# EspressoSystems/Push-CDN

Measured on NVIDIA H100. Metric: broadcast fan-out egress GB/s (1 KiB x 2^20 subscribers per GPU, 1 topic); msgs/s and % of HBM peak alongside, higher is better.
Workload: dtype u8

## Files before the change

push-cdn_b200/csrc/kernels.cu:

```cuda
#include "kernels.cuh"

#include <atomic>

#include "frame_parse_core.h"

namespace pcdn {

std::atomic<unsigned long long> g_kernel_launches{0};
#define PCDN_COUNT_LAUNCH (void)g_kernel_launches.fetch_add(1, std::memory_order_relaxed)

unsigned long long kernel_launches() { return g_kernel_launches.load(std::memory_order_relaxed); }
void count_kernel_launch() { PCDN_COUNT_LAUNCH; }

__device__ __forceinline__ uint32_t lane_id() { return threadIdx.x & 31; }

__device__ __forceinline__ uint32_t warp_incl_scan(uint32_t v) {
  const uint32_t lane = lane_id();
#pragma unroll
  for (int o = 1; o < 32; o <<= 1) {
    uint32_t n = __shfl_up_sync(0xffffffffu, v, o);
    if (lane >= (uint32_t)o) v += n;
  }
  return v;
}
// ... 649 lines not shown
      }
    } else if (threadIdx.x == 0) {
      cta_prefix = 0;
      w.lb_tot[vb] = ctot;
    }
    __syncthreads();
    k.s1_off = cta_prefix + cex;
    w.cbase[c] = k.s1_off;
  } else {
    s.ptail[c] = k.pt;
    s.used[c] = k.us;
  }
  w.batch_units[c] = k.bu;

  const uint32_t nsp = (k.s1_rec ? 1u : 0u) + (k.s2_rec ? 1u : 0u);
  uint32_t tot, ex;
  uint32_t run_len = 1, my_runs = nsp, nsp_warp = 0;
  if (s.span_runs) {
    __shared__ uint32_t r_off[NT], r_len[NT], r_rec[NT], r_brk[NT + 1];
    const uint32_t t = threadIdx.x;
    r_off[t] = k.s1_off; r_len[t] = k.s1_units; r_rec[t] = nsp == 1 ? k.s1_rec : 0u;
    __syncthreads();
    const bool cont = t > 0 && nsp == 1 && r_rec[t - 1] == k.s1_rec && r_len[t - 1] == k.s1_units &&
                      (s.pool ? r_off[t - 1] + r_len[t - 1] == k.s1_off : r_off[t - 1] == k.s1_off);
    const uint32_t head = (nsp > 0 && !cont) ? 1u : 0u;
    my_runs = head ? nsp : 0u;
    uint32_t ptot;
    const uint32_t pex = cta_excl_scan<NW>(my_runs | (cont ? 0u : 1u << 16), &ptot, sm);
    ex = pex & 0xFFFFu; tot = ptot & 0xFFFFu;
    const uint32_t brk = pex >> 16;
    if (!cont) r_brk[brk] = t;
    if (t == 0) r_brk[ptot >> 16] = NT;
    __syncthreads();
    if (head) run_len = r_brk[brk + 1] - t;
    if (threadIdx.x == 0) span_base = tot ? atomicAdd(&w.stats->n_runs, tot) : 0;
    nsp_warp = __reduce_add_sync(0xffffffffu, nsp);
  } else {
    ex = cta_excl_scan<NW>(nsp, &tot, sm);
    if (threadIdx.x == 0) span_base = tot ? atomicAdd(&w.stats->n_spans, tot) : 0;
  }
  const unsigned long long nrec = __reduce_add_sync(0xffffffffu, k.s1_rec + k.s2_rec);
  const unsigned long long by = (unsigned long long)__reduce_add_sync(0xffffffffu, k.bytes & 0xFFFFu) +
                                ((unsigned long long)__reduce_add_sync(0xffffffffu, k.bytes >> 16) << 16);
  if (lane == 0) { red[0][threadIdx.x >> 5] = nrec | ((unsigned long long)nsp_warp << 48); red[1][threadIdx.x >> 5] = by; }
  __syncthreads();
  if (threadIdx.x == 0) {
    unsigned long long a = 0, bb = 0, sp = 0;
    for (int i = 0; i < NW; i++) { a += red[0][i] & 0xFFFFFFFFFFFFull; sp += red[0][i] >> 48; bb += red[1][i]; }
    if (a) { atomicAdd(&w.stats->n_deliveries, a); atomicAdd(&w.stats->bytes_out, bb); }
    if (sp) atomicAdd(&w.stats->n_spans, (uint32_t)sp);
  }
  if (s.span_runs) {
    if (my_runs) {
      SpanRun* runs = reinterpret_cast<SpanRun*>(w.spans);
      uint32_t at = span_base + ex;
      if (k.s1_rec) runs[at++] = SpanRun{s.conn_base + c, run_len, s.pool ? k.s1_off : k.s1_off * kUnit, k.s1_units * kUnit, k.s1_rec, s.pool ? k.s1_units : 0u};
      if (k.s2_rec) runs[at] = SpanRun{s.conn_base + c, 1, 0, k.s2_units * kUnit, k.s2_rec, 0};
    }
  } else if (nsp) {
    uint32_t at = span_base + ex;
    if (k.s1_rec) w.spans[at++] = Span{s.conn_base + c, s.pool ? k.s1_off : k.s1_off * kUnit, k.s1_units * kUnit, k.s1_rec};
    if (k.s2_rec) w.spans[at] = Span{s.conn_base + c, 0, k.s2_units * kUnit, k.s2_rec};
  }
  if (k.ovf) {
    uint32_t i = atomicAdd(&w.stats->n_overflow, 1u);
    if (i < max_conns) w.overflow[i] = s.conn_base + c;
  }
}
template <bool HAS_DIRECT>
__global__ void __launch_bounds__(256) k_offsets(DevState s, BatchIn b, Work w, uint32_t max_conns) {
  offsets_body<HAS_DIRECT, 256, false, false>(s, b, w, max_conns, blockIdx.x * 256 + threadIdx.x, blockIdx.x, gridDim.x);
}
__global__ void __launch_bounds__(1024) k_pool_finish(DevState s, Work w, uint32_t nblk) {
  extern __shared__ uint32_t tb[];
  __shared__ uint32_t sm[33];
  __shared__ unsigned long long total_s;
  if (w.stats->status) return;
  unsigned long long carry = 0;
  for (uint32_t b0 = 0; b0 < nblk; b0 += 1024) {
    const uint32_t i = b0 + threadIdx.x;
    const uint32_t v = i < nblk ? w.lb_tot[i] : 0;
    uint32_t tot, ex = cta_excl_scan<32>(v, &tot, sm);
    const unsigned long long at = carry + ex;
    if (i < nblk) tb[i] = at > 0xFFFFFFFFull ? 0xFFFFFFFFu : (uint32_t)at;
    carry += tot;
  }
  if (threadIdx.x == 0) total_s = carry;
  __syncthreads();
  if (blockIdx.x == 0 && threadIdx.x == 0) pool_allocate(s, w, total_s);
  const uint32_t gt = blockIdx.x * 1024 + threadIdx.x, gn = gridDim.x * 1024;
  for (uint32_t c = gt; c < s.N; c += gn) w.cbase[c] += tb[c >> 8];
  if (s.span_runs) {
    SpanRun* r = reinterpret_cast<SpanRun*>(w.spans);
    const uint32_t n = w.stats->n_runs;
    for (uint32_t i = gt; i < n; i += gn) r[i].ring_off += tb[(r[i].conn0 - s.conn_base) >> 8];
  } else {
    const uint32_t n = w.stats->n_spans;
    for (uint32_t i = gt; i < n; i += gn) w.spans[i].ring_off += tb[(w.spans[i].conn - s.conn_base) >> 8];
  }
}

void launch_offsets(const DevState& s, const Work& w, const BatchIn& b, bool has_direct, int n_sms, cudaStream_t st) {
  if (has_direct) PCDN_COUNT_LAUNCH, k_offsets<true><<<s.N / 256, 256, 0, st>>>(s, b, w, s.N);
  else PCDN_COUNT_LAUNCH, k_offsets<false><<<s.N / 256, 256, 0, st>>>(s, b, w, s.N);
  if (s.pool) {
    const uint32_t nblk = s.N / 256;
    if (nblk * 4 > 48u * 1024) cudaFuncSetAttribute(k_pool_finish, cudaFuncAttributeMaxDynamicSharedMemorySize, (int)(nblk * 4));
    PCDN_COUNT_LAUNCH, k_pool_finish<<<std::min<uint32_t>((uint32_t)n_sms, (s.N + 8191) / 8192), 1024, nblk * 4, st>>>(s, w, nblk);
  }
}

__device__ __forceinline__ void cluster_sync_all() {
  asm volatile("barrier.cluster.arrive.release.aligned;\n\tbarrier.cluster.wait.acquire.aligned;" ::: "memory");
}
template <bool HAS_DIRECT>
__global__ void __cluster_dims__(8, 1, 1) __launch_bounds__(1024, 1)
k_ctrl_small(DevState s, BatchIn b, Work w, int zero_stats, BatchStats* publish, int offsets_only) {
  __shared__ uint32_t sm[33];
  __shared__ uint32_t gbase[5];
  const uint32_t tid = threadIdx.x, rank = blockIdx.x;
  if (zero_stats && rank == 0 && tid < sizeof(BatchStats) / 4) reinterpret_cast<uint32_t*>(w.stats)[tid] = 0;

  if (HAS_DIRECT && rank == 0 && !offsets_only) {
    __shared__ uint32_t skey_s[kSmallCtrlMsgs], sorted_s[kSmallCtrlMsgs];
    __syncthreads();
    for (uint32_t g0 = 0; g0 < b.n_msgs * 8; g0 += 1024) direct_lookup_body<false>(s, b, w, g0 + tid);
    __syncthreads();
    const uint32_t n = b.n_msgs;
    if (tid < n) { const uint32_t t = w.dconn[tid]; skey_s[tid] = t == kConnNone ? s.N : t; }
    __syncthreads();
    if (tid < n) {
      const uint32_t key = skey_s[tid];
      uint32_t r = 0;
      for (uint32_t o = 0; o < n; o++) r += (skey_s[o] < key || (skey_s[o] == key && o < tid)) ? 1u : 0u;
      sorted_s[r] = key;
      w.dlist[r] = tid;
    }
    __syncthreads();
    if (tid < n) {
      const uint32_t key = sorted_s[tid];
      if (tid == 0 || sorted_s[tid - 1] != key) { w.dstart[key] = tid; w.dstamp[key] = w.stamp; }
      if (tid + 1 == n || sorted_s[tid + 1] != key) w.dend[key] = tid + 1;
    }
  }

  if (!offsets_only) {
    const uint32_t q = tid >> 8, wl = tid & 255u, nitems = b.n_bcast * s.nblk;
    for (uint32_t i0 = rank * 4; i0 < nitems; i0 += 32) {
      const uint32_t it = i0 + q;
      const bool live = it < nitems;
      const uint32_t j = live ? it / s.nblk : 0, blk = live ? it % s.nblk : 0;
      const uint32_t wd = blk * kBlockWords + wl;
      const uint32_t word = live ? match_word(s, b, b.bcast_index[j], wd) : 0;
      uint32_t tot, ex = cta_excl_scan<32>(__popc(word), &tot, sm);
      if (wl == 0) gbase[q] = ex;
      if (tid == 0) gbase[4] = tot;
      __syncthreads();
      if (live) {
        w.B[(size_t)j * s.W + wd] = word;
        w.wpre[(size_t)j * s.W + wd] = (uint16_t)(ex - gbase[q]);
        if (wl == 0) w.cnt[(size_t)j * s.nblk + blk] = gbase[q + 1] - gbase[q];
      }
      __syncthreads();
    }
  }
  cluster_sync_all();

  if (rank == 0 && !offsets_only) {
    if (tid < b.n_bcast) {
      uint32_t carry = 0;
      for (uint32_t blk = 0; blk < s.nblk; blk++) {
        const uint32_t v = w.cnt[(size_t)tid * s.nblk + blk];
        w.base[(size_t)tid * s.nblk + blk] = carry;
        carry += v;
      }
      const uint32_t m = b.bcast_index[tid];
      w.D[m] = carry; w.jidx[m] = tid;
    }
    __syncthreads();
  }

  if (rank == 0 && !offsets_only) {
    const uint32_t m = tid;
    const bool valid = m < b.n_msgs;
    const uint32_t d = valid ? w.D[m] : 0;
    uint32_t cls, tiles;
    plan_classify(s, b, m, d, &cls, &tiles);
    uint32_t t0, t1, t2, t3;
    const uint32_t e0 = cta_excl_scan<32>(cls != CLS_THIN ? d : 0, &t0, sm);
    const uint32_t e1 = cta_excl_scan<32>(cls == CLS_THIN ? d : 0, &t1, sm);
    const uint32_t e2 = cta_excl_scan<32>(tiles, &t2, sm);
    const uint32_t e3 = cta_excl_scan<32>(cls == CLS_CM ? 1u : 0u, &t3, sm);
    if (valid) {
      w.eb_fat[m] = e0; w.eb_thin[m] = e1; w.tbase[m] = e2; w.cm_rank[m] = e3; w.cls[m] = (uint8_t)cls;
      if (cls == CLS_CM) w.cm_list[e3] = m;
    }
    if (tid == 0) {
      w.stats->n_fat_entries = t0; w.stats->n_thin_entries = t1; w.stats->n_fat_tiles = t2; w.stats->tile_cursor = 0;
      w.stats->n_cm = t3; w.stats->cm_cursor = 0;
      if (t0 > w.cap_fat || t1 > w.cap_thin) w.stats->status = 1;
      const uint32_t n = b.n_msgs;
      w.eb_fat[n] = t0; w.eb_thin[n] = t1; w.tbase[n] = t2; w.cm_rank[n] = t3;
    }
  }
  cluster_sync_all();

  for (uint32_t c0 = 0; c0 < s.N; c0 += 8192)
    offsets_body<HAS_DIRECT, 1024, true, true>(s, b, w, s.N, c0 + rank * 1024 + tid, c0 / 1024 + rank, s.N / 1024);

  if (publish) {
    cluster_sync_all();
    if (rank == 0 && tid < sizeof(BatchStats) / 4)
      reinterpret_cast<uint32_t*>(publish)[tid] = __ldcg(reinterpret_cast<const uint32_t*>(w.stats) + tid);
  }
}
void launch_ctrl_small(const DevState& s, const Work& w, const BatchIn& b, bool has_direct, bool zero_stats,
                       BatchStats* publish, bool offsets_only, cudaStream_t st) {
  if (has_direct) PCDN_COUNT_LAUNCH, k_ctrl_small<true><<<8, 1024, 0, st>>>(s, b, w, zero_stats ? 1 : 0, publish, offsets_only ? 1 : 0);
  else PCDN_COUNT_LAUNCH, k_ctrl_small<false><<<8, 1024, 0, st>>>(s, b, w, zero_stats ? 1 : 0, publish, offsets_only ? 1 : 0);
}

__global__ void k_pool_retry_begin(BatchStats* bs) {
  bs->status = 0;
  bs->n_deliveries = 0; bs->bytes_out = 0;
  bs->n_spans = 0; bs->n_runs = 0; bs->n_overflow = 0;
  bs->tile_cursor = 0; bs->cm_cursor = 0;
}
void launch_pool_retry_begin(const DevState& s, const Work& w, cudaStream_t st) {
  cudaMemsetAsync(w.lb_state, 0, ((size_t)s.N / 256 + 1) * 8, st);
  PCDN_COUNT_LAUNCH, k_pool_retry_begin<<<1, 1, 0, st>>>(w.stats);
}

__device__ __forceinline__ uint8_t* conn_out(const DevState& s, const Work& w, uint32_t conn, uint32_t pool_base) {
  return s.pool ? s.rings + ((size_t)pool_base + w.cbase[conn]) * kUnit : s.rings + (size_t)conn * s.ring_bytes;
}

__device__ __forceinline__ void pack_fat_phase(const DevState& s, const BatchIn& b, const Work& w, uint8_t* buf,
                                               uint64_t* barp) {
  uint64_t& bar = *barp;
  __shared__ uint32_t t_info[8];
  const uint32_t tid = threadIdx.x;
  const uint32_t ntiles = w.stats->n_fat_tiles;
  if (ntiles == 0) return;
  const uint32_t pool_base = w.stats->pool_base;
  uint32_t phase = 0;
  uint32_t staged_m = 0xFFFFFFFFu, staged_k = 0xFFFFFFFFu;

  for (;;) {
    if (tid == 0) {
      const uint32_t t = atomicAdd(&w.stats->tile_cursor, 1u);
      t_info[0] = t;
      if (t < ntiles) {
        uint32_t lo = 0, hi = b.n_msgs;
        while (hi - lo > 1) { uint32_t mid = (lo + hi) >> 1; if (w.tbase[mid] <= t) lo = mid; else hi = mid; }
        const uint32_t m = lo, ltile = t - w.tbase[m], d = w.D[m];
        const uint32_t fb = frame_vec_bytes(b.raw_len[m]);
        const uint32_t tr = tile_recipients(fb);
        const uint32_t ngrp = (d + tr - 1) / tr;
        const uint32_t ch = ltile / ngrp, grp = ltile % ngrp;
        const uint32_t nbytes = min(kChunkBytes, fb - ch * kChunkBytes);
        t_info[1] = m; t_info[2] = ch; t_info[3] = grp * tr;
        t_info[4] = min(d, (grp + 1) * tr); t_info[5] = nbytes;
        t_info[6] = (m != staged_m || ch != staged_k) ? 1u : 0u;
        staged_m = m; staged_k = ch;
      }
    }
    __syncthreads();
    if (t_info[0] >= ntiles) break;
    const uint32_t m = t_info[1], ch = t_info[2], r0 = t_info[3], r1 = t_info[4], nbytes = t_info[5];
    if (t_info[6]) {
      bulk_wait_read0();
      __syncthreads();
      if (tid == 0) {
        mbar_arrive_expect_tx(&bar, nbytes);
        bulk_g2s(buf, b.arena + (size_t)b.slot_off16[m] * 16 + (size_t)ch * kChunkBytes, nbytes, &bar);
      }
      mbar_wait(&bar, phase);
      phase ^= 1;
      if (ch == 0) {
        if (tid == 0) {
          *reinterpret_cast<uint32_t*>(buf) = bswap32(b.raw_len[m]);
          fence_proxy_async_smem();
        }
        __syncthreads();
      }
    }
    const uint2* E = w.efat + w.eb_fat[m];
    const size_t chunk_off = (size_t)ch * kChunkBytes;
    for (uint32_t r = r0 + tid; r < r1; r += 256) {
      const uint2 ent = E[r];
      if (ent.y != kOffInvalid)
        bulk_s2g(conn_out(s, w, ent.x, pool_base) + (size_t)ent.y * kUnit + chunk_off, buf, nbytes);
    }
    bulk_commit();
    __syncthreads();
  }
  bulk_wait_read0();
}

__device__ __forceinline__ void pack_cm_phase(const DevState& s, const BatchIn& b, const Work& w, uint8_t* buf,
                                              uint64_t* barp) {
  uint64_t& bar = *barp;
  __shared__ uint32_t g_m[kCmGroup], g_j[kCmGroup], g_soff[kCmGroup], g_units[kCmGroup], g_eb[kCmGroup];
  __shared__ uint32_t t_info[4];
  const uint32_t tid = threadIdx.x, lane = tid & 31, warp = tid >> 5;
  if (w.stats->status) return;
  const uint32_t ncm = w.stats->n_cm;
  if (ncm == 0) return;
  const uint32_t pool_base = w.stats->pool_base;
  const uint32_t ngroups = (ncm + kCmGroup - 1) / kCmGroup;
  const uint32_t tpg = s.W / kCmTileWords;
  const uint32_t ntiles = ngroups * tpg;
  uint32_t phase = 0;
  uint32_t staged_g = 0xFFFFFFFFu;

  for (;;) {
    if (tid == 0) {
      const uint32_t t = atomicAdd(&w.stats->cm_cursor, 1u);
      t_info[0] = t;
      if (t < ntiles) {
        const uint32_t g = t / tpg;
        const uint32_t gcount = min(kCmGroup, ncm - g * kCmGroup);
        t_info[1] = g; t_info[2] = gcount;
        t_info[3] = g != staged_g ? 1u : 0u;
        staged_g = g;
      }
    }
    __syncthreads();
    if (t_info[0] >= ntiles) break;
    const uint32_t gcount = t_info[2];
    if (t_info[3]) {
      bulk_wait_read0();
      __syncthreads();
      if (tid == 0) {
        const uint32_t g = t_info[1];
        uint32_t soff = 0, total = 0;
        for (uint32_t i = 0; i < gcount; i++) {
          const uint32_t m = w.cm_list[g * kCmGroup + i];
          const uint32_t len = b.raw_len[m];
          g_m[i] = m; g_j[i] = w.jidx[m]; g_soff[i] = soff; g_units[i] = frame_units(len); g_eb[i] = w.eb_fat[m];
          soff += frame_units(len) * kUnit;
          total += frame_vec_bytes(len);
        }
        mbar_arrive_expect_tx(&bar, total);
        for (uint32_t i = 0; i < gcount; i++)
          bulk_g2s(buf + g_soff[i], b.arena + (size_t)b.slot_off16[g_m[i]] * 16, frame_vec_bytes(b.raw_len[g_m[i]]), &bar);
      }
      __syncthreads();
      mbar_wait(&bar, phase);
      phase ^= 1;
      if (tid < gcount) {
        *reinterpret_cast<uint32_t*>(buf + g_soff[tid]) = bswap32(b.raw_len[g_m[tid]]);
        fence_proxy_async_smem();
      }
      __syncthreads();
    }
    const uint32_t wt = t_info[0] % tpg;
    for (uint32_t wi = warp; wi < kCmTileWords; wi += 8) {
      const uint32_t wd = wt * kCmTileWords + wi;
      const uint32_t myword = lane < gcount ? w.B[(size_t)g_j[lane] * s.W + wd] : 0u;
      const uint32_t any = __reduce_or_sync(0xffffffffu, myword);
      if (!any) continue;
      uint32_t offs[kCmGroup];
#pragma unroll
      for (int i = 0; i < (int)kCmGroup; i++) {
        const uint32_t wordi = __shfl_sync(0xffffffffu, myword, i);
        offs[i] = kOffInvalid;
        if ((uint32_t)i < gcount && ((wordi >> lane) & 1u)) {
          const uint32_t j = g_j[i];
          const uint32_t idx = g_eb[i] + w.base[(size_t)j * s.nblk + wd / kBlockWords] + w.wpre[(size_t)j * s.W + wd] +
                               __popc(wordi & ((1u << lane) - 1u));
          offs[i] = w.ecm[idx];
        }
      }
      uint8_t* ring = conn_out(s, w, wd * 32 + lane, pool_base);
      uint32_t run_o = kOffInvalid, run_units = 0, run_s = 0;
#pragma unroll
      for (int i = 0; i < (int)kCmGroup; i++) {
        const uint32_t o = offs[i];
        if (o != kOffInvalid && run_o != kOffInvalid && o == run_o + run_units) {
          run_units += g_units[i];
        } else {
          if (run_o != kOffInvalid) bulk_s2g(ring + (size_t)run_o * kUnit, buf + run_s, run_units * kUnit);
          run_o = o; run_s = g_soff[i]; run_units = (o != kOffInvalid) ? g_units[i] : 0;
        }
      }
      if (run_o != kOffInvalid) bulk_s2g(ring + (size_t)run_o * kUnit, buf + run_s, run_units * kUnit);
    }
    bulk_commit();
    __syncthreads();
  }
  bulk_wait_read0();
}

__device__ __forceinline__ void copy_record(const uint4* __restrict__ src, uint4* __restrict__ dst, uint32_t raw_len, uint32_t lane) {
  const uint32_t nvec = (4u + raw_len + 15u) >> 4;
  const uint32_t hdr = bswap32(raw_len);
  for (uint32_t v = lane; v < nvec; v += 128) {
    uint4 x0, x1, x2, x3;
    const bool p1 = v + 32 < nvec, p2 = v + 64 < nvec, p3 = v + 96 < nvec;
    x0 = ld_nc16(src + v);
    if (p1) x1 = ld_nc16(src + v + 32);
    if (p2) x2 = ld_nc16(src + v + 64);
    if (p3) x3 = ld_nc16(src + v + 96);
    if (v == 0) x0.x = hdr;
    st_stream16(dst + v, x0);
    if (p1) st_stream16(dst + v + 32, x1);
    if (p2) st_stream16(dst + v + 64, x2);
    if (p3) st_stream16(dst + v + 96, x3);
  }
}
__device__ __forceinline__ void pack_thin_phase(const DevState& s, const BatchIn& b, const Work& w) {
  const uint32_t n = w.stats->n_thin_entries;
  const uint32_t pool_base = w.stats->pool_base;
  const uint32_t lane = lane_id();
  const uint32_t gw = (blockIdx.x * blockDim.x + threadIdx.x) >> 5, nw = (gridDim.x * blockDim.x) >> 5;
  for (uint32_t e = gw; e < n; e += nw) {
    const uint4 ent = w.ethin[e];
    if (ent.y == kOffInvalid) continue;
    copy_record(reinterpret_cast<const uint4*>(b.arena + (size_t)ent.z * 16),
                reinterpret_cast<uint4*>(conn_out(s, w, ent.x, pool_base) + (size_t)ent.y * kUnit), ent.w, lane);
  }
}
__device__ __forceinline__ void pack_direct_phase(const DevState& s, const BatchIn& b, const Work& w) {
  const uint32_t n = b.n_msgs;
  const uint32_t pool_base = w.stats->pool_base;
  const uint32_t lane = lane_id();
  const uint32_t gw = (blockIdx.x * blockDim.x + threadIdx.x) >> 5, nw = (gridDim.x * blockDim.x) >> 5;
  uint2 ent = make_uint2(0, kOffInvalid);
  uint32_t so = 0, len = 0;
  if (gw < n) { ent = w.edir[gw]; so = b.slot_off16[gw]; len = b.raw_len[gw]; }
  for (uint32_t m = gw; m < n; m += nw) {
    const uint2 cur = ent;
    const uint32_t cso = so, clen = len;
    const uint32_t nx = m + nw;
    if (nx < n) { ent = w.edir[nx]; so = b.slot_off16[nx]; len = b.raw_len[nx]; }
    if (cur.y == kOffInvalid) continue;
    copy_record(reinterpret_cast<const uint4*>(b.arena + (size_t)cso * 16),
                reinterpret_cast<uint4*>(conn_out(s, w, cur.x, pool_base) + (size_t)cur.y * kUnit), clen, lane);
  }
}

__global__ void __launch_bounds__(256) k_pack(DevState s, BatchIn b, Work w, int do_direct) {
  __shared__ __align__(128) uint8_t buf[kCmGroup * kCmMaxBytes];
  __shared__ __align__(8) uint64_t bars[2];
  if (w.stats->status) return;
  if (threadIdx.x == 0) {
    mbar_init(&bars[0], 1);
    mbar_init(&bars[1], 1);
    asm volatile("fence.mbarrier_init.release.cluster;" ::: "memory");
  }
  __syncthreads();
  pack_cm_phase(s, b, w, buf, &bars[0]);
  __syncthreads();
  pack_fat_phase(s, b, w, buf, &bars[1]);
  pack_thin_phase(s, b, w);
  if (do_direct) pack_direct_phase(s, b, w);
}
__global__ void __launch_bounds__(256, 8) k_pack_direct(DevState s, BatchIn b, Work w) {
  if (w.stats->status) return;
  pack_direct_phase(s, b, w);
}

__device__ __forceinline__ void st_ref_record(uint8_t* dst, uint32_t raw_len, uint32_t slot_off16, unsigned long long batch_id) {
  const unsigned long long off = (unsigned long long)slot_off16 * 16u + 4u;
  st_stream16(dst, make_uint4(0xFFFFFFFFu, bswap32(raw_len), (uint32_t)off, (uint32_t)(off >> 32)));
  st_stream16(dst + 16, make_uint4((uint32_t)batch_id, (uint32_t)(batch_id >> 32), 0u, 0u));
}
__global__ void __launch_bounds__(256) k_pack_ref(DevState s, BatchIn b, Work w, int do_direct) {
  if (w.stats->status) return;
  const uint32_t nfat = w.stats->n_fat_entries, nthin = w.stats->n_thin_entries;
  const uint64_t nft = (uint64_t)nfat + nthin, total = nft + (do_direct ? b.n_msgs : 0u);
  const uint32_t pool_base = w.stats->pool_base;
  const unsigned long long bid = w.batch_id;
  const uint64_t stride = (uint64_t)gridDim.x * blockDim.x;
  for (uint64_t i = (uint64_t)blockIdx.x * blockDim.x + threadIdx.x; i < total; i += stride) {
    uint32_t conn, off, m = 0, slot = 0, len = 0;
    bool thin = false;
    if (i < nfat) {
      const uint32_t e = (uint32_t)i;
      uint32_t lo = 0, hi = b.n_msgs;
      while (hi - lo > 1) { const uint32_t mid = (lo + hi) >> 1; if (w.eb_fat[mid] <= e) lo = mid; else hi = mid; }
      const uint2 ent = w.efat[e];
      conn = ent.x; off = ent.y; m = lo;
    } else if (i < nft) {
      const uint4 ent = w.ethin[i - nfat];
      conn = ent.x; off = ent.y; slot = ent.z; len = ent.w; thin = true;
    } else {
      m = (uint32_t)(i - nft);
      const uint2 ent = w.edir[m];
      conn = ent.x; off = ent.y;
    }
    if (off == kOffInvalid) continue;
    if (!thin) { slot = b.slot_off16[m]; len = b.raw_len[m]; }
    st_ref_record(conn_out(s, w, conn, pool_base) + (size_t)off * kUnit, len, slot, bid);
  }
}

void launch_pack(const DevState& s, const Work& w, const BatchIn& b, uint32_t n_direct, uint32_t pack_variant, int n_sms, cudaStream_t st) {
  if (s.shared_payload) {
    if (b.n_bcast || n_direct) PCDN_COUNT_LAUNCH, k_pack_ref<<<(uint32_t)n_sms * 8, 256, 0, st>>>(s, b, w, n_direct ? 1 : 0);
    return;
  }
  const bool direct_separate = n_direct >= kThinSeparateMin;
  const uint32_t ctas_per_sm = ((pack_variant >> 8) & 15u) ? ((pack_variant >> 8) & 15u) : 3;
  const uint32_t grid = (uint32_t)n_sms * ctas_per_sm;
  const int do_direct = (n_direct && !direct_separate) ? 1 : 0;
  if (b.n_bcast || do_direct)
    PCDN_COUNT_LAUNCH, k_pack<<<grid, 256, 0, st>>>(s, b, w, do_direct);
  const uint32_t dctas = ((pack_variant >> 12) & 15u) ? ((pack_variant >> 12) & 15u) : 8u;
  if (direct_separate) PCDN_COUNT_LAUNCH, k_pack_direct<<<(uint32_t)n_sms * dctas, 256, 0, st>>>(s, b, w);
}

__global__ void __launch_bounds__(256) k_release(DevState s, const uint32_t* __restrict__ batch_units,
                                                 const BatchStats* __restrict__ stats) {
  if (stats->status) return;
  const uint32_t i = blockIdx.x * blockDim.x + threadIdx.x;
  if (i * 4 < s.N) {
    const uint4 u = reinterpret_cast<const uint4*>(batch_units)[i];
    if (u.x | u.y | u.z | u.w) {
      uint4* p = reinterpret_cast<uint4*>(s.used) + i;
      uint4 v = *p;
      v.x -= u.x; v.y -= u.y; v.z -= u.z; v.w -= u.w;
      *p = v;
    }
  }
}
__global__ void k_pool_release(PoolState* p, const BatchStats* __restrict__ stats) {
  if (stats->status) return;
  p->used -= stats->pool_units + stats->pool_skip;
  p->tail = stats->pool_base + stats->pool_units;
  if (p->used == 0) { p->head = 0; p->tail = 0; }
}
__global__ void k_pool_init(PoolState* p) { p->head = 0; p->tail = 0; p->used = 0; p->blocked = 0; }
void launch_pool_init(const DevState& s, cudaStream_t st) {
  if (s.pool) PCDN_COUNT_LAUNCH, k_pool_init<<<1, 1, 0, st>>>(s.pool_state);
}
void launch_release(const DevState& s, const uint32_t* batch_units, const BatchStats* stats, cudaStream_t st) {
  if (s.pool) { PCDN_COUNT_LAUNCH, k_pool_release<<<1, 1, 0, st>>>(s.pool_state, stats); return; }
  PCDN_COUNT_LAUNCH, k_release<<<(s.N / 4 + 255) / 256, 256, 0, st>>>(s, batch_units, stats);
}

}
```

Before: 2930.

## Prefetch next CM tile, parallelize group staging, batch per-warp word lookups

Restructures the coalesced-multicast packing loop. The next tile is claimed with an atomic before the current tile is processed and published through a double-buffered t_info, which removes one barrier per tile. Group metadata staging and TMA issue move from a single thread to a warp, using a scan for the shared-memory offsets. Each warp now unrolls over all its tile words, issuing the bitmap and index loads for every word before the dependent ecm gathers, to expose more memory-level parallelism. The cost is higher register pressure from the offs[k][i] arrays, and it relies on kCmTileWords dividing evenly by 8.

```diff
diff --git a/push-cdn_b200/csrc/kernels.cu b/push-cdn_b200/csrc/kernels.cu
--- a/push-cdn_b200/csrc/kernels.cu
+++ b/push-cdn_b200/csrc/kernels.cu
@@ -975,7 +975,9 @@
                                               uint64_t* barp) {
   uint64_t& bar = *barp;
   __shared__ uint32_t g_m[kCmGroup], g_j[kCmGroup], g_soff[kCmGroup], g_units[kCmGroup], g_eb[kCmGroup];
-  __shared__ uint32_t t_info[4];
+  __shared__ uint32_t t_info[2][4];
+  constexpr uint32_t kWordsPerWarp = kCmTileWords / 8;
+  static_assert(kCmTileWords % 8 == 0, "a tile is split evenly over the 8 warps");
   const uint32_t tid = threadIdx.x, lane = tid & 31, warp = tid >> 5;
   if (w.stats->status) return;
   const uint32_t ncm = w.stats->n_cm;
@@ -986,38 +988,40 @@
   const uint32_t ntiles = ngroups * tpg;
   uint32_t phase = 0;
   uint32_t staged_g = 0xFFFFFFFFu;
-
-  for (;;) {
-    if (tid == 0) {
-      const uint32_t t = atomicAdd(&w.stats->cm_cursor, 1u);
-      t_info[0] = t;
-      if (t < ntiles) {
-        const uint32_t g = t / tpg;
-        const uint32_t gcount = min(kCmGroup, ncm - g * kCmGroup);
-        t_info[1] = g; t_info[2] = gcount;
-        t_info[3] = g != staged_g ? 1u : 0u;
-        staged_g = g;
-      }
-    }
-    __syncthreads();
-    if (t_info[0] >= ntiles) break;
-    const uint32_t gcount = t_info[2];
-    if (t_info[3]) {
+  auto publish = [&](uint32_t* ti, uint32_t t) {
+    ti[0] = t;
+    if (t < ntiles) {
+      const uint32_t g = t / tpg;
+      ti[1] = g; ti[2] = min(kCmGroup, ncm - g * kCmGroup);
+      ti[3] = g != staged_g ? 1u : 0u;
+      staged_g = g;
+    }
+  };
+  if (tid == 0) publish(t_info[0], atomicAdd(&w.stats->cm_cursor, 1u));
+  __syncthreads();
+
+  for (uint32_t cb = 0;; cb ^= 1u) {
+    const uint32_t t = t_info[cb][0];
+    if (t >= ntiles) break;
+    const uint32_t gcount = t_info[cb][2];
+    if (t_info[cb][3]) {
       bulk_wait_read0();
       __syncthreads();
-      if (tid == 0) {
-        const uint32_t g = t_info[1];
-        uint32_t soff = 0, total = 0;
-        for (uint32_t i = 0; i < gcount; i++) {
-          const uint32_t m = w.cm_list[g * kCmGroup + i];
-          const uint32_t len = b.raw_len[m];
-          g_m[i] = m; g_j[i] = w.jidx[m]; g_soff[i] = soff; g_units[i] = frame_units(len); g_eb[i] = w.eb_fat[m];
-          soff += frame_units(len) * kUnit;
-          total += frame_vec_bytes(len);
+      if (warp == 0) {
+        const uint32_t g = t_info[cb][1];
+        uint32_t m = 0, len = 0, u = 0;
+        if (lane < gcount) {
+          m = w.cm_list[g * kCmGroup + lane];
+          len = b.raw_len[m];
+          u = frame_units(len);
+          g_m[lane] = m; g_j[lane] = w.jidx[m]; g_units[lane] = u; g_eb[lane] = w.eb_fat[m];
         }
-        mbar_arrive_expect_tx(&bar, total);
-        for (uint32_t i = 0; i < gcount; i++)
-          bulk_g2s(buf + g_soff[i], b.arena + (size_t)b.slot_off16[g_m[i]] * 16, frame_vec_bytes(b.raw_len[g_m[i]]), &bar);
+        const uint32_t soff = warp_incl_scan(u * kUnit) - u * kUnit;
+        const uint32_t total = __reduce_add_sync(0xffffffffu, lane < gcount ? frame_vec_bytes(len) : 0u);
+        if (lane < gcount) g_soff[lane] = soff;
+        if (lane == 0) mbar_arrive_expect_tx(&bar, total);
+        __syncwarp();
+        if (lane < gcount) bulk_g2s(buf + soff, b.arena + (size_t)b.slot_off16[m] * 16, frame_vec_bytes(len), &bar);
       }
       __syncthreads();
       mbar_wait(&bar, phase);
@@ -1028,29 +1032,39 @@
       }
       __syncthreads();
     }
-    const uint32_t wt = t_info[0] % tpg;
-    for (uint32_t wi = warp; wi < kCmTileWords; wi += 8) {
-      const uint32_t wd = wt * kCmTileWords + wi;
-      const uint32_t myword = lane < gcount ? w.B[(size_t)g_j[lane] * s.W + wd] : 0u;
-      const uint32_t any = __reduce_or_sync(0xffffffffu, myword);
-      if (!any) continue;
-      uint32_t offs[kCmGroup];
+    uint32_t next = 0;
+    if (tid == 0) next = atomicAdd(&w.stats->cm_cursor, 1u);
+    const uint32_t wt = t % tpg;
+    uint32_t myword[kWordsPerWarp], offs[kWordsPerWarp][kCmGroup];
+    bool any[kWordsPerWarp];
+#pragma unroll
+    for (uint32_t k = 0; k < kWordsPerWarp; k++) {
+      const uint32_t wd = wt * kCmTileWords + warp + 8 * k;
+      myword[k] = lane < gcount ? w.B[(size_t)g_j[lane] * s.W + wd] : 0u;
 #pragma unroll
       for (int i = 0; i < (int)kCmGroup; i++) {
-        const uint32_t wordi = __shfl_sync(0xffffffffu, myword, i);
-        offs[i] = kOffInvalid;
-        if ((uint32_t)i < gcount && ((wordi >> lane) & 1u)) {
-          const uint32_t j = g_j[i];
-          const uint32_t idx = g_eb[i] + w.base[(size_t)j * s.nblk + wd / kBlockWords] + w.wpre[(size_t)j * s.W + wd] +
-                               __popc(wordi & ((1u << lane) - 1u));
-          offs[i] = w.ecm[idx];
-        }
-      }
-      uint8_t* ring = conn_out(s, w, wd * 32 + lane, pool_base);
+        const uint32_t j = g_j[i];
+        offs[k][i] = (uint32_t)i < gcount ? g_eb[i] + w.base[(size_t)j * s.nblk + wd / kBlockWords] + w.wpre[(size_t)j * s.W + wd] : 0u;
+      }
+    }
+#pragma unroll
+    for (uint32_t k = 0; k < kWordsPerWarp; k++) {
+      any[k] = __reduce_or_sync(0xffffffffu, myword[k]) != 0;
+#pragma unroll
+      for (int i = 0; i < (int)kCmGroup; i++) {
+        const uint32_t wordi = __shfl_sync(0xffffffffu, myword[k], i);
+        const bool hit = (uint32_t)i < gcount && ((wordi >> lane) & 1u);
+        offs[k][i] = hit ? w.ecm[offs[k][i] + __popc(wordi & ((1u << lane) - 1u))] : kOffInvalid;
+      }
+    }
+#pragma unroll
+    for (uint32_t k = 0; k < kWordsPerWarp; k++) {
+      if (!any[k]) continue;
+      uint8_t* ring = conn_out(s, w, (wt * kCmTileWords + warp + 8 * k) * 32 + lane, pool_base);
       uint32_t run_o = kOffInvalid, run_units = 0, run_s = 0;
 #pragma unroll
       for (int i = 0; i < (int)kCmGroup; i++) {
-        const uint32_t o = offs[i];
+        const uint32_t o = offs[k][i];
         if (o != kOffInvalid && run_o != kOffInvalid && o == run_o + run_units) {
           run_units += g_units[i];
         } else {
@@ -1061,6 +1075,7 @@
       if (run_o != kOffInvalid) bulk_s2g(ring + (size_t)run_o * kUnit, buf + run_s, run_units * kUnit);
     }
     bulk_commit();
+    if (tid == 0) publish(t_info[cb ^ 1u], next);
     __syncthreads();
   }
   bulk_wait_read0();
```

New measurement: 2978, median of 6. +1.6%, better.
